# zraorg/ZRA

Hardware: AMD Instinct MI355X
Metric: compress + RA-decompress GiB/s, 16 GiB @ 64 KiB frames, 1/2/4/8 MI355X (higher is better)
Workload: dtype u8

## Files before the change

zra_amd/csrc/zra_encode.hip:

```cpp
#include <cstdio>
#include <unistd.h>
#include "zra_host.h"
#include "zra_dev.h"
#include "zra_format.h"
#include "zra_env.h"
#include <algorithm>
#include <cstdlib>
#include <vector>

extern "C" __global__ void zra_mf_kernel(ZraEncArgs a, uint32_t block, uint32_t only, uint32_t onlySlot, uint32_t perWave);
extern "C" __global__ void zra_mf_opt_kernel(ZraEncArgs a, uint32_t block, uint32_t only, uint32_t onlySlot, uint32_t perWave);
extern "C" __global__ void zra_mf_dfast_ls_kernel(ZraEncArgs a, uint32_t block, uint32_t only, uint32_t onlySlot);
extern "C" __global__ void zra_mf_hc_kernel(ZraEncArgs a, uint32_t block, uint32_t only, uint32_t onlySlot);
extern "C" __global__ void zra_mf_fast_kernel(ZraEncArgs a, uint32_t block, uint32_t perWave);
extern "C" __global__ void zra_mf_dfast_kernel(ZraEncArgs a, uint32_t block, uint32_t only, uint32_t onlySlot);
extern "C" __global__ void zra_mf_dfast_fl_kernel(ZraEncArgs a, ZraFlagArgs g, uint32_t block, uint32_t only, uint32_t onlySlot);
extern "C" __global__ void zra_entropy_kernel(ZraEncArgs a, uint32_t block);
extern "C" __global__ void zra_entropy_front_kernel(ZraEncArgs a, uint32_t block);
extern "C" __global__ void zra_entropy_back_kernel(ZraEncArgs a, uint32_t block);
extern "C" __global__ void zra_ent_chain_kernel(ZraEncArgs a);
extern "C" __global__ void zra_ent_chain5_kernel(ZraEncArgs a);

using namespace zra_dev;
using namespace zra_env;
// ... 147 lines not shown
      if (!encScan_.reserve(64)) return zerr(64);
      bool okProbe = hipMemsetAsync(encScan_.p, 0, 64, stream2_) == hipSuccess &&
                     hipStreamWaitValue32(stream2_, encScan_.p, 0, hipStreamWaitValueGte, 0xFFFFFFFFu) == hipSuccess &&
                     hipStreamSynchronize(stream2_) == hipSuccess;
      if (!okProbe) (void)hipGetLastError();
      waitValueOk_ = okProbe ? 1 : -1;
    }
    if (waitValueOk_ < 0) persist = false;
    if (persist)
      return compress_persistent(dIn, inSize, dBody, bodyBase0, dEntries, dSizes, bodySize, frameSize, checksum, full, tail,
                                 tableWords, seqStride, litStride, slotStride);
  }
  uint64_t budget = 8ull << 30;
  if (env_set("ZRA_ENC_BUDGET_GIB")) budget = (uint64_t)env_int("ZRA_ENC_BUDGET_GIB", 0) << 30;
  else if (full.strategy != 2) {
    size_t freeB = 0, totalB = 0;
    uint64_t mine = 0; for (auto& x : encCtx_) mine += x.tables.cap + x.seqs.cap + x.lits.cap + x.slots.cap;
    if (hipMemGetInfo(&freeB, &totalB) == hipSuccess) budget = std::min<uint64_t>(64ull << 30, std::max<uint64_t>(budget, (uint64_t)(((uint64_t)freeB + mine) * 0.25)));
  }
  uint32_t B = (uint32_t)std::max<uint64_t>(1, std::min<uint64_t>({nFramesTotal, budget / perFrame, full.strategy == 2 ? 16384ull : 65536ull}));
  if (B > 1024) B &= ~1023u;
  { uint64_t nBatches = (nFramesTotal + B - 1) / B;
    if (maxBlocksPerFrame > 1 && nBatches == 1 && nFramesTotal >= 32ull * (uint64_t)numCUs_) nBatches = 2;
    if (nBatches > 1) B = (uint32_t)std::min<uint64_t>(B, ((nFramesTotal + nBatches - 1) / nBatches + 63) & ~63ull); }
  const uint32_t entGridB = (uint32_t)std::min<uint64_t>(B, (uint64_t)numCUs_ * 5);
  const uint64_t entWorkStride = (9 * seqStride + 255) & ~255ull;
  const int nCtx = nFramesTotal > B ? 2 : 1;
  for (int c = 0; c < nCtx; c++) {
    EncCtx& x = encCtx_[c];
    if (!x.tables.reserve(B * tableWords * 4) || !x.seqs.reserve(B * seqStride * 8) || !x.lits.reserve((size_t)entGridB * litStride) ||
        !x.work.reserve((size_t)entGridB * entWorkStride) ||
        !x.slots.reserve(B * slotStride) || !x.misc.reserve(B * (sizeof(ZraEncFrameState) + sizeof(ZraEncBlockOut))) ||
        !x.ck.reserve((size_t)B * 4) || !x.sizes.reserve((size_t)B * 16))
      return zerr(64);
  }
  const size_t nEntLaunches = (size_t)((nFramesTotal + B - 1) / B) * maxBlocksPerFrame + 4;
  if (!encScan_.reserve(64 + 4 * nEntLaunches)) return zerr(64);
  uint64_t* dRunning = encScan_.as<uint64_t>();
  uint32_t* dEntQueues = (uint32_t*)(encScan_.as<uint8_t>() + 64);
  HIPCHK(hipMemsetAsync(encScan_.p, 0, 64 + 4 * nEntLaunches, stream2_));
  size_t entLaunch = 0;

  ZraEncArgs base{};
  base.in = dIn; base.inSize = inSize; base.frameSize = frameSize; base.checksum = checksum ? 1 : 0;
  base.full = full; base.tail = tail;
  dbgSeqStride_ = seqStride; dbgB_ = (uint32_t)B;
  base.tableStride = tableWords; base.seqStride = seqStride; base.litStride = litStride; base.slotStride = slotStride;
  base.entWorkStride = entWorkStride; base.slotRing = B; base.entSubFrames = B; base.entPrio = 3;

  size_t evNext = 0;
  auto ev = [&]() -> hipEvent_t {
    if (evNext == evPool_.size()) { hipEvent_t e = nullptr; if (hipEventCreate(&e) != hipSuccess) return nullptr; evPool_.push_back(e); }
    return evPool_[evNext++];
  };
  std::vector<std::pair<hipEvent_t, hipEvent_t>> mfSpans, entSpans;
  hipEvent_t entDone[2] = {nullptr, nullptr};
  hipStream_t mfStream2 = nullptr;
  if (nCtx == 2) {
    if (!pipeStreams_[0] && hipStreamCreateWithFlags(&pipeStreams_[0], hipStreamNonBlocking) != hipSuccess) { pipeStreams_[0] = nullptr; (void)hipGetLastError(); }
    mfStream2 = pipeStreams_[0];
  }
  { hipEvent_t e0 = ev(); if (!e0) return zerr(1); HIPCHK(hipEventRecord(e0, stream_)); HIPCHK(hipStreamWaitEvent(stream2_, e0, 0));
    if (mfStream2) HIPCHK(hipStreamWaitEvent(mfStream2, e0, 0)); }

  uint64_t batchIdx = 0;
  for (uint64_t f0 = 0; f0 < nFramesTotal; f0 += B, batchIdx++) {
    const uint32_t nb = (uint32_t)std::min<uint64_t>(B, nFramesTotal - f0);
    const int c = (int)(batchIdx % nCtx);
    EncCtx& x = encCtx_[c];
    ZraEncArgs a = base;
    a.firstFrame = (uint32_t)f0; a.nFrames = nb;
    a.tables = x.tables.as<uint32_t>(); a.seqs = x.seqs.as<uint64_t>(); a.lits = x.lits.as<uint8_t>(); a.slots = x.slots.as<uint8_t>();
    a.state = x.misc.as<ZraEncFrameState>();
    a.blockOut = (ZraEncBlockOut*)(x.misc.as<uint8_t>() + (size_t)B * sizeof(ZraEncFrameState));
    a.contentCk = x.ck.as<uint32_t>();
    a.sizes = x.sizes.as<uint64_t>();
    uint64_t* dOffsets = x.sizes.as<uint64_t>() + B;
    if (checksum)
      hipLaunchKernelGGL(zra_content_ck_kernel, dim3((nb * 4 + 255) / 256), dim3(256), 0, stream2_, dIn, (u64)inSize, frameSize, (u32)f0, nb, a.contentCk);
    const uint64_t firstFrameSize = std::min<uint64_t>(frameSize, inSize - f0 * frameSize);
    const ZraEncParams& P0 = firstFrameSize == frameSize ? full : tail;
    const uint32_t rounds = (uint32_t)((firstFrameSize + P0.blockSize - 1) / P0.blockSize);
    hipStream_t sA = (c == 1 && mfStream2) ? mfStream2 : stream_;
    if (entDone[c]) HIPCHK(hipStreamWaitEvent(sA, entDone[c], 0));
    { static const bool poison = env_set("ZRA_ENC_POISON");
      if (poison) HIPCHK(hipMemsetAsync(x.tables.p, 0xA5, (size_t)nb * tableWords * 4, sA)); }
    for (uint32_t blk = 0; blk < rounds; blk++) {
      hipEvent_t m0 = ev(), m1 = ev(), e1 = ev();
      if (!m0 || !m1 || !e1) return zerr(1);
      HIPCHK(hipEventRecord(m0, sA));
      {
        const bool hasTail = tailSize && f0 + nb == nFramesTotal;
        const uint32_t shL = 1, shS = 2, dupLog = 8;
        a.mfFilter = shL | (shS << 4) | (dupLog << 8);
        const uint32_t hl = std::max(full.hashLog, tail.hashLog), cl = std::max(full.chainLog, tail.chainLog);
        const size_t filterBytes = (8u << dupLog) + (((size_t)1 << hl) >> shL) / 8 + (((size_t)1 << cl) >> shS) / 8 + 64;
        const bool serialAll = std::min<uint64_t>(frameSize, inSize) > (1ull << full.windowLog);
        a.serialAll = serialAll ? 1u : 0u;
        const bool oddTail = !serialAll && hasTail && (tail.strategy == 2) != (full.strategy == 2);
        auto launchLone = [&](uint32_t only, uint32_t slot) {
          if (tail.strategy >= 3 && tail.strategy <= 5) hipLaunchKernelGGL(zra_mf_hc_kernel, dim3(1), dim3(64), 0, sA, a, blk, only, slot);
          else hipLaunchKernelGGL(mfGeneric, dim3(1), dim3(64), 0, sA, a, blk, only, slot, 1u);
        };
        if (full.strategy == 2 && !serialAll) {
          hipLaunchKernelGGL(zra_mf_dfast_kernel, dim3(nb), dim3(64), filterBytes, sA, a, blk, 0xFFFFFFFFu, 0u);
          if (oddTail) launchLone((uint32_t)(nb - 1), (uint32_t)(nb - 1));
        } else {
          const bool hashChain = full.strategy >= 3 && full.strategy <= 5 && !serialAll;
          const uint32_t perWave = hashChain ? 1u : std::min<uint32_t>(8u, std::max<uint32_t>(1u, (nb + (uint32_t)numCUs_ * 32 - 1) / ((uint32_t)numCUs_ * 32)));
          const bool lean = hashChain || full.strategy == 1;
          const uint32_t hcPad = hashChain && full.searchLog >= 5 && tableWords * 4 >= (4ull << 20) ? 5120u : 0u;
          if (hashChain) hipLaunchKernelGGL(zra_mf_hc_kernel, dim3(nb), dim3(64), hcPad, sA, a, blk, 0xFFFFFFFFu, 0u);
          else if (lean) hipLaunchKernelGGL(zra_mf_fast_kernel, dim3((nb + perWave - 1) / perWave), dim3(64), 0, sA, a, blk, perWave);
          else hipLaunchKernelGGL(mfGeneric, dim3((nb + perWave - 1) / perWave), dim3(64), 0, sA, a, blk, 0xFFFFFFFFu, 0u, perWave);
          if (oddTail) hipLaunchKernelGGL(zra_mf_dfast_kernel, dim3(1), dim3(64), filterBytes, sA, a, blk, (uint32_t)(nb - 1), (uint32_t)(nb - 1));
          else if (lean && hasTail && (hashChain ? (tail.strategy < 3 || tail.strategy > 5) : tail.strategy != 1))
            launchLone((uint32_t)(nb - 1), (uint32_t)(nb - 1));
        }
      }
      HIPCHK(hipEventRecord(m1, sA));
      mfSpans.push_back({m0, m1});
      HIPCHK(hipStreamWaitEvent(stream2_, m1, 0));
      hipEvent_t e0 = ev(); if (!e0) return zerr(1);
      HIPCHK(hipEventRecord(e0, stream2_));
      { ZraEncArgs ae = a; ae.entQueue = dEntQueues + entLaunch++; ae.entWork = x.work.as<uint8_t>();
        hipLaunchKernelGGL(zra_entropy_kernel, dim3(std::min<uint32_t>(nb, entGridB)), dim3(256), 0, stream2_, ae, blk); }
      HIPCHK(hipEventRecord(e1, stream2_));
      entSpans.push_back({e0, e1});
      if (blk + 1 < rounds) HIPCHK(hipStreamWaitEvent(sA, e1, 0));
    }
    hipLaunchKernelGGL(zra_scan_sizes_kernel, dim3(1), dim3(64), 0, stream2_, a.sizes, nb, dOffsets, dRunning, (const u32*)nullptr);
    hipLaunchKernelGGL(zra_gather_frames_kernel, dim3(nb), dim3(256), 0, stream2_, a.slots, slotStride, a.sizes, dOffsets, dBody,
                       bodyBase0, dEntries ? dEntries : nullptr, (u32)f0, dSizes, (const u32*)nullptr);
    hipEvent_t done = ev(); if (!done) return zerr(1);
    HIPCHK(hipEventRecord(done, stream2_));
    entDone[c] = done;
    if ((uint64_t)env_i64("ZRA_ENC_FAIL_BATCH", -1) == batchIdx) return zerr(1);
  }
  uint64_t total = 0;
  HIPCHK(hipMemcpyAsync(&total, dRunning, 8, hipMemcpyDeviceToHost, stream2_));
  HIPCHK(hipStreamSynchronize(stream2_));
  HIPCHK(hipStreamSynchronize(stream_));
  if (mfStream2) HIPCHK(hipStreamSynchronize(mfStream2));
  HIPCHK(hipGetLastError());
  double kernelMs = 0;
  kstats_[0] = kstats_[1] = kstats_[2] = kstats_[3] = 0;
  for (auto& sp : mfSpans) { float m = 0; if (hipEventElapsedTime(&m, sp.first, sp.second) == hipSuccess) { kstats_[0] += m; kstats_[1] += 1; kernelMs += m; } }
  for (auto& sp : entSpans) { float m = 0; if (hipEventElapsedTime(&m, sp.first, sp.second) == hipSuccess) { kstats_[2] += m; kstats_[3] += 1; } }
  lastKernelMs_ = kernelMs;
  *bodySize = total;
  return ok();
}

Status Engine::compress_persistent(const uint8_t* dIn, size_t inSize, uint8_t* dBody, uint64_t bodyBase0, uint8_t* dEntries, uint64_t* dSizes,
                                   size_t* bodySize, uint32_t frameSize, bool checksum, const ZraEncParams& full, const ZraEncParams& tail,
                                   uint64_t tableWords, uint64_t seqStride, uint64_t litStride, uint64_t slotStride) {
  const uint64_t nFramesTotal = (inSize + frameSize - 1) / frameSize;
  const size_t tailSize = inSize % frameSize;
  const auto mfGeneric = (full.strategy >= 7 || tail.strategy >= 7) ? zra_mf_opt_kernel : zra_mf_kernel;
  static const uint32_t wavesPerCU = (uint32_t)env_int("ZRA_MF_WAVES", 19);
  constexpr uint32_t SB = 8192;
  const uint32_t nSlots = (uint32_t)std::min<uint64_t>((uint64_t)numCUs_ * wavesPerCU, nFramesTotal);
  const uint64_t perFrame = seqStride * 8 + sizeof(ZraEncFrameState) + sizeof(ZraEncBlockOut) + 4 + 16 + 8;
  uint64_t budget;
  {
    size_t freeB = 0, totalB = 0;
    if (hipMemGetInfo(&freeB, &totalB) != hipSuccess) freeB = 24ull << 30;
    uint64_t mine = 0; for (auto& x : encCtx_) mine += x.seqs.cap;
    budget = std::min<uint64_t>(64ull << 30, std::max<uint64_t>(8ull << 30, ((uint64_t)freeB + mine) / 3));
  }
  uint64_t SBIG = 0, nSuper = 0, subsPerSuper = 0; int nCtx = 1;
  EncCtx& sh = encCtx_[0];
  static const uint32_t entPerCU = (uint32_t)std::max(1, env_int("ZRA_ENT_WGS", 8));
  const uint32_t entGrid = (uint32_t)std::min<uint64_t>((uint64_t)numCUs_ * entPerCU, nFramesTotal);
  const uint64_t entWorkStride = (9 * seqStride + 255) & ~255ull;
  static const int splitEnv = env_int("ZRA_ENT_SPLIT", 1);
  const bool entSplit = splitEnv >= 2 || (splitEnv == 1 && nFramesTotal >= 256);
  uint64_t slotRing = 0;
  for (;; budget /= 2) {
    SBIG = std::max<uint64_t>(1, std::min<uint64_t>(nFramesTotal, budget / perFrame));
    if (SBIG > SB) SBIG -= SBIG % SB;
    nCtx = nFramesTotal > SBIG ? 2 : 1;
    nSuper = (nFramesTotal + SBIG - 1) / SBIG;
    subsPerSuper = (SBIG + SB - 1) / SB;
    slotRing = std::min<uint64_t>(SB, SBIG);
    const uint64_t workUnits = entSplit ? std::min<uint64_t>(SB, nFramesTotal) : entGrid;
    bool okR = sh.tables.reserve((size_t)nSlots * tableWords * 4) && sh.lits.reserve((size_t)entGrid * litStride) && sh.work.reserve((size_t)workUnits * entWorkStride) &&
               sh.slots.reserve(slotRing * slotStride) && (!entSplit || sh.rec.reserve((size_t)workUnits * sizeof(ZraEntRec)));
    for (int c = 0; c < nCtx && okR; c++) {
      EncCtx& x = encCtx_[c];
      okR = x.seqs.reserve(SBIG * seqStride * 8) && x.misc.reserve(SBIG * (sizeof(ZraEncFrameState) + sizeof(ZraEncBlockOut))) &&
            x.ck.reserve((size_t)SBIG * 4) && x.sizes.reserve((size_t)SBIG * 16);
    }
    if (okR) break;
    if (budget <= (1ull << 30) || SBIG <= SB) return zerr(64);
    (void)hipGetLastError();
  }
  const size_t nCnt = 4 + 8 * (size_t)nSuper + 4 * (size_t)(nSuper * subsPerSuper) + 4;
  const size_t cntCore = (16 + 4 * nCnt + 15) & ~(size_t)15;
  const size_t cntBytes = cntCore + 8 * (size_t)ZRA_TELE_WORDS;
  if (!encScan_.reserve(cntBytes)) return zerr(64);
  uint64_t* dRunning = encScan_.as<uint64_t>();
  uint32_t* dCnt = (uint32_t*)(encScan_.as<uint8_t>() + 16);
  uint32_t* dPerSuper = dCnt + 4;
  uint32_t* dPerSub = dPerSuper + 8 * nSuper;
  HIPCHK(hipMemsetAsync(encScan_.as<uint8_t>(), 0, cntBytes, stream_));
  encCounters_ = dCnt; encCountersBytes_ = 4 * (4 + 8 * (size_t)nSuper + 4 * (size_t)(nSuper * subsPerSuper));

  ZraEncArgs base{};
  base.in = dIn; base.inSize = inSize; base.frameSize = frameSize; base.checksum = checksum ? 1 : 0;
  base.full = full; base.tail = tail;
  dbgSeqStride_ = seqStride; dbgB_ = (uint32_t)SBIG;
  base.tableStride = tableWords; base.seqStride = seqStride; base.litStride = litStride; base.slotStride = slotStride;
  base.mfTele = (uint64_t*)(encScan_.as<uint8_t>() + cntCore);
  base.entWorkStride = entWorkStride;
  base.entPrio = 1;
  base.entSubFrames = SB; base.slotRing = (uint32_t)slotRing; base.readyStamp = 1u;
  const uint32_t shL = 1, shS = 3, dupLog = 8;
  base.mfFilter = shL | (shS << 4) | (dupLog << 8);
  const uint32_t hl = std::max(full.hashLog, tail.hashLog), cl = std::max(full.chainLog, tail.chainLog);
  const size_t filterBytes = (8u << dupLog) + (((size_t)1 << hl) >> shL) / 8 + (((size_t)1 << cl) >> shS) / 8;

  static const int lsEnv = env_int("ZRA_MF_LS", 1);
  const uint32_t lsBytes = (uint32_t)((std::min<uint64_t>(frameSize, inSize) + 64 + 63) & ~63ull);
  const uint32_t lsPerCu = (uint32_t)((160u << 10) / (lsBytes + filterBytes));
  static const int lsMaxEnv = env_int("ZRA_MF_LS_MAX", -1);
  bool useLs = lsEnv != 0 && full.strategy == 2 && lsPerCu >= 1 &&
               nFramesTotal <= (lsMaxEnv >= 0 ? (uint64_t)lsMaxEnv : (uint64_t)lsPerCu * (uint64_t)numCUs_);
  if (useLs && lsAttr_ == 0) {
    const bool okA = hipFuncSetAttribute((const void*)zra_mf_dfast_ls_kernel, hipFuncAttributeMaxDynamicSharedMemorySize, 160 << 10) == hipSuccess;
    if (!okA) (void)hipGetLastError();
    lsAttr_ = okA ? 1 : -1;
  }
  if (lsAttr_ < 0) useLs = false;

  static const int flEnv = env_int("ZRA_MF_FLAGS", 1);
  const bool useFlagsWave = flEnv != 0 && !useLs && full.strategy == 2;
  ZraFlagArgs fw{};
  if (useFlagsWave) {
    fw.flagStride = ((((uint64_t)std::min<uint64_t>(frameSize, inSize) + 511) / 512) * 128 + 255) & ~255ull;
    if (!mfFlags_.reserve((size_t)nSlots * fw.flagStride)) return zerr(64);
    fw.flags = mfFlags_.as<uint8_t>(); fw.ldsWords = (uint32_t)(filterBytes / 4);
    fw.spanBytes = 768;
    static const int epEnv = env_int("ZRA_MF_EPOCH", 4);
    const uint32_t ibMax = 32u - (uint32_t)__builtin_clz((uint32_t)std::max<uint64_t>(2, std::min<uint64_t>(frameSize, inSize)) - 1u);
    fw.epochBits = (uint32_t)std::max(0, std::min(epEnv, (int)(32u - ibMax) - 10));
  }
  const size_t spanLds = fw.spanBytes ? fw.spanBytes + 16 + (fw.spanBytes / 64 + 1) * 16 : 0;

  size_t evNext = 0;
  auto ev = [&]() -> hipEvent_t {
    if (evNext == evPool_.size()) { hipEvent_t e = nullptr; if (hipEventCreate(&e) != hipSuccess) return nullptr; evPool_.push_back(e); }
    return evPool_[evNext++];
  };
  std::vector<std::pair<hipEvent_t, hipEvent_t>> mfSpans, entSpans;
  static const bool traceOn = env_set("ZRA_ENC_TRACE");
  hipEvent_t superDone[2] = {nullptr, nullptr};
  { hipEvent_t e0 = ev(); if (!e0) return zerr(1); HIPCHK(hipEventRecord(e0, stream_)); HIPCHK(hipStreamWaitEvent(stream2_, e0, 0)); }

  for (uint64_t S = 0; S < nSuper; S++) {
    const uint64_t F0 = S * SBIG;
    const uint32_t n = (uint32_t)std::min<uint64_t>(SBIG, nFramesTotal - F0);
    const int c = (int)(S % nCtx);
    EncCtx& x = encCtx_[c];
    ZraEncArgs a = base;
    a.firstFrame = (uint32_t)F0; a.nFrames = n;
    a.tables = sh.tables.as<uint32_t>(); a.lits = sh.lits.as<uint8_t>(); a.slots = sh.slots.as<uint8_t>(); a.entWork = sh.work.as<uint8_t>();
    a.seqs = x.seqs.as<uint64_t>();
    a.state = x.misc.as<ZraEncFrameState>();
    a.blockOut = (ZraEncBlockOut*)(x.misc.as<uint8_t>() + (size_t)SBIG * sizeof(ZraEncFrameState));
    a.contentCk = x.ck.as<uint32_t>();
    a.sizes = x.sizes.as<uint64_t>();
    a.mfQueue = dPerSuper + 8 * S; a.mfStarted = a.mfQueue + 1;
    uint32_t* const entQ = dPerSub + 4 * S * subsPerSuper;
    a.mfDone = entQ + 3 * subsPerSuper;
    if (superDone[c]) HIPCHK(hipStreamWaitEvent(stream_, superDone[c], 0));
    HIPCHK(hipMemsetAsync(a.blockOut, 0, (size_t)n * sizeof(ZraEncBlockOut), stream_));
    hipEvent_t m0 = ev(), m1 = ev();
    if (!m0 || !m1) return zerr(1);
    HIPCHK(hipEventRecord(m0, stream_));
    const uint32_t mfGrid = std::min<uint32_t>(n, nSlots);
    if (useFlagsWave) hipLaunchKernelGGL(zra_mf_dfast_fl_kernel, dim3(mfGrid), dim3(64), filterBytes + spanLds, stream_, a, fw, 0u, 0xFFFFFFFFu, 0u);
    else if (useLs) {
      ZraEncArgs al = a; al.mfFilter |= (lsBytes / 64) << 16;
      hipLaunchKernelGGL(zra_mf_dfast_ls_kernel, dim3(mfGrid), dim3(64), lsBytes + filterBytes, stream_, al, 0u, 0xFFFFFFFFu, 0u);
    } else hipLaunchKernelGGL(zra_mf_dfast_kernel, dim3(mfGrid), dim3(64), filterBytes, stream_, a, 0u, 0xFFFFFFFFu, 0u);
    HIPCHK(hipGetLastError());
    HIPCHK(hipEventRecord(m1, stream_));
    mfSpans.push_back({m0, m1});
    const bool oddTail = tailSize && F0 + n == nFramesTotal && tail.strategy != 2;
    if (oddTail) {
      ZraEncArgs at = a; at.mfQueue = nullptr;
      if (tail.strategy >= 3 && tail.strategy <= 5) hipLaunchKernelGGL(zra_mf_hc_kernel, dim3(1), dim3(64), 0, stream_, at, 0u, (uint32_t)(n - 1), 0u);
      else hipLaunchKernelGGL(mfGeneric, dim3(1), dim3(64), 0, stream_, at, 0u, (uint32_t)(n - 1), 0u, 1u);
    }
    HIPCHK(hipStreamWaitValue32(stream2_, a.mfStarted, mfGrid, hipStreamWaitValueGte, 0xFFFFFFFFu));
    if (checksum)
      hipLaunchKernelGGL(zra_content_ck_kernel, dim3((n * 4 + 255) / 256), dim3(256), 0, stream2_, dIn, (u64)inSize, frameSize, (u32)F0, n, a.contentCk);
    const uint32_t nSub1 = (n + SB - 1) / SB;
    for (uint32_t j = 0; j < nSub1; j++) {
      const uint32_t j0 = j * SB, nbj = std::min<uint32_t>(SB, n - j0);
      const bool hasOdd = oddTail && j == nSub1 - 1;
      HIPCHK(hipStreamWaitValue32(stream2_, a.mfDone + j, nbj - (hasOdd ? 1u : 0u), hipStreamWaitValueGte, 0xFFFFFFFFu));
      if (hasOdd) { hipEvent_t te = ev(); if (!te) return zerr(1); HIPCHK(hipEventRecord(te, stream_)); HIPCHK(hipStreamWaitEvent(stream2_, te, 0)); }
      ZraEncArgs aj = a;
      aj.firstFrame = (uint32_t)(F0 + j0); aj.nFrames = nbj;
      aj.seqs = a.seqs + (size_t)j0 * seqStride; aj.state = a.state + j0; aj.blockOut = a.blockOut + j0;
      aj.contentCk = a.contentCk + j0; aj.sizes = a.sizes + j0;
      aj.entQueue = entQ + j;
      uint64_t* dOffsets = x.sizes.as<uint64_t>() + SBIG + j0;
      hipEvent_t e0 = ev(), e1 = ev(); if (!e0 || !e1) return zerr(1);
      HIPCHK(hipEventRecord(e0, stream2_));
      if (entSplit) {
        aj.entRec = sh.rec.as<ZraEntRec>();
        hipLaunchKernelGGL(zra_entropy_front_kernel, dim3(std::min<uint32_t>(nbj, entGrid)), dim3(256), 0, stream2_, aj, 0u);
        const uint32_t cg = wavesPerCU >= 19 ? 5u : 6u;
        hipLaunchKernelGGL(cg == 5 ? zra_ent_chain5_kernel : zra_ent_chain_kernel, dim3((nbj + cg - 1) / cg), dim3(64), 0, stream2_, aj);
        ZraEncArgs ab = aj; ab.entQueue = entQ + subsPerSuper + j;
        hipLaunchKernelGGL(zra_entropy_back_kernel, dim3(std::min<uint32_t>(nbj, entGrid)), dim3(256), 0, stream2_, ab, 0u);
      } else
        hipLaunchKernelGGL(zra_entropy_kernel, dim3(std::min<uint32_t>(nbj, entGrid)), dim3(256), 0, stream2_, aj, 0u);
      HIPCHK(hipEventRecord(e1, stream2_));
      entSpans.push_back({e0, e1});
      hipLaunchKernelGGL(zra_scan_sizes_kernel, dim3(1), dim3(64), 0, stream2_, aj.sizes, nbj, dOffsets, dRunning, (const u32*)nullptr);
      hipLaunchKernelGGL(zra_gather_frames_kernel, dim3(nbj), dim3(256), 0, stream2_, aj.slots, slotStride, aj.sizes, dOffsets, dBody,
                         bodyBase0, dEntries ? dEntries : nullptr, (u32)(F0 + j0), dSizes, (const u32*)nullptr);
    }
    hipEvent_t done = ev(); if (!done) return zerr(1);
    HIPCHK(hipEventRecord(done, stream2_));
    superDone[c] = done;
  }
  uint64_t total = 0;
  HIPCHK(hipMemcpyAsync(&total, dRunning, 8, hipMemcpyDeviceToHost, stream2_));
  HIPCHK(hipStreamSynchronize(stream2_));
  HIPCHK(hipStreamSynchronize(stream_));
  HIPCHK(hipGetLastError());
  double kernelMs = 0;
  kstats_[0] = kstats_[1] = kstats_[2] = kstats_[3] = 0;
  for (auto& sp : mfSpans) { float m = 0; if (hipEventElapsedTime(&m, sp.first, sp.second) == hipSuccess) { kstats_[0] += m; kstats_[1] += 1; kernelMs += m; } }
  for (auto& sp : entSpans) { float m = 0; if (hipEventElapsedTime(&m, sp.first, sp.second) == hipSuccess) { kstats_[2] += m; kstats_[3] += 1; } }
  lastKernelMs_ = kernelMs;
  mfTeleDev_ = base.mfTele;
  if (traceOn) {
    for (auto& sp : mfSpans) { float a0 = 0, a1 = 0; (void)hipEventElapsedTime(&a0, mfSpans[0].first, sp.first); (void)hipEventElapsedTime(&a1, mfSpans[0].first, sp.second); std::fprintf(stderr, "mf  %8.2f .. %8.2f ms\n", a0, a1); }
    for (auto& sp : entSpans) { float a0 = 0, a1 = 0; (void)hipEventElapsedTime(&a0, mfSpans[0].first, sp.first); (void)hipEventElapsedTime(&a1, mfSpans[0].first, sp.second); std::fprintf(stderr, "ent %8.2f .. %8.2f ms\n", a0, a1); }
  }
  *bodySize = total;
  return ok();
}

size_t Engine::launch_telemetry(uint64_t* out, size_t cap) {
  if (mfTeleDev_) {
    (void)hipSetDevice(device_);
    mfTele_.resize(ZRA_TELE_HEAD + 8 + ZRA_TELE_CUKEYS);
    const bool okT = hipMemcpy(mfTele_.data(), mfTeleDev_, 8 * (size_t)ZRA_TELE_HEAD, hipMemcpyDeviceToHost) == hipSuccess &&
                     hipMemcpy(mfTele_.data() + ZRA_TELE_HEAD, mfTeleDev_ + ZRA_TELE_ENT, 8 * (size_t)(8 + ZRA_TELE_CUKEYS), hipMemcpyDeviceToHost) == hipSuccess;
    if (!okT) { (void)hipGetLastError(); mfTele_.clear(); }
    mfTeleDev_ = nullptr;
  }
  const size_t n = mfTele_.size() < cap ? mfTele_.size() : cap;
  for (size_t i = 0; i < n; i++) out[i] = mfTele_[i];
  return n;
}

uint32_t Engine::debug_read_seqs(uint32_t frame, uint64_t* out, uint32_t cap, uint32_t meta[3]) {
  if (!dbgB_ || frame >= dbgB_) return 0;
  (void)hipSetDevice(device_);
  (void)hipDeviceSynchronize();
  EncCtx& x = encCtx_[0];
  ZraEncBlockOut bo{};
  (void)hipMemcpy(&bo, x.misc.as<uint8_t>() + (size_t)dbgB_ * sizeof(ZraEncFrameState) + (size_t)frame * sizeof(ZraEncBlockOut), sizeof(bo), hipMemcpyDeviceToHost);
  meta[0] = bo.nbSeq; meta[1] = bo.lastLL; meta[2] = bo.skip;
  const uint32_t n = bo.nbSeq < cap ? bo.nbSeq : cap;
  if (n) (void)hipMemcpy(out, x.seqs.as<uint64_t>() + (size_t)frame * dbgSeqStride_, (size_t)n * 8, hipMemcpyDeviceToHost);
  return n;
}

Status Engine::compress_device(const uint8_t* dIn, size_t inSize, uint8_t* dOut, size_t* outSize, int level, uint32_t frameSize, bool checksum) {
  HIPCHK(hipSetDevice(device_));
  if (frameSize == 0) return zerr(42);
  const uint32_t tableSize = zra_fmt::table_size(inSize, frameSize);
  const size_t headerSize = zra_fmt::kFixedSize + (size_t)tableSize * zra_fmt::kEntrySize;
  size_t bodySize = 0;
  Status s = compress_impl(dIn, inSize, dOut + headerSize, 0, dOut + zra_fmt::kFixedSize, nullptr, &bodySize, level, frameSize, checksum);
  if (s.zra) return s;
  if (headerSize + bodySize >= zra_fmt::kMaxCompressedSize) return {kCompressedTooLarge, 0};
  std::vector<uint8_t> hdr(headerSize);
  if (tableSize > 1)
    HIPCHK(hipMemcpyAsync(hdr.data() + zra_fmt::kFixedSize, dOut + zra_fmt::kFixedSize, (size_t)(tableSize - 1) * 5, hipMemcpyDeviceToHost, stream_));
  HIPCHK(hipStreamSynchronize(stream_));
  zra_fmt::write_fixed(hdr.data(), inSize, tableSize, frameSize, 0);
  zra_fmt::entry_put(hdr.data() + zra_fmt::kFixedSize + (size_t)(tableSize - 1) * 5, bodySize);
  zra_fmt::wr32(hdr.data() + 14, zra_fmt::header_hash(hdr.data(), hdr.data() + zra_fmt::kFixedSize));
  HIPCHK(hipMemcpyAsync(dOut, hdr.data(), zra_fmt::kFixedSize, hipMemcpyHostToDevice, stream_));
  HIPCHK(hipMemcpyAsync(dOut + zra_fmt::kFixedSize + (size_t)(tableSize - 1) * 5, hdr.data() + zra_fmt::kFixedSize + (size_t)(tableSize - 1) * 5, 5,
                        hipMemcpyHostToDevice, stream_));
  HIPCHK(hipStreamSynchronize(stream_));
  *outSize = headerSize + bodySize;
  return ok();
}

// ... 21 lines not shown
```

zra_amd/csrc/zra_encode_mf.hip:

```cpp
#include "zra_dev.h"
#include "zra_kernels.h"
#include "zra_encode_wave.h"

using namespace zra_dev;
using namespace zra_wave;

#ifdef ZRA_MF_PROFILE
__device__ unsigned long long zra_mf_prof[24];
#define PROF_DECL u64 pt_[20]; for (int k_ = 0; k_ < 20; k_++) pt_[k_] = 0; u64 pl_ = __builtin_amdgcn_s_memtime();
#define PROF(k) { __builtin_amdgcn_s_waitcnt(0); const u64 n_ = __builtin_amdgcn_s_memtime(); pt_[k] += n_ - pl_; pl_ = n_; }
#define PROF_CNT(k) { pt_[k]++; }
#define PROF_END { if (lane == 0) for (int k_ = 0; k_ < 20; k_++) atomicAdd(&zra_mf_prof[k_], pt_[k_]); }
#elif defined(ZRA_MF_MARK)
#define PROF_DECL
#define PROF(k) asm volatile("; ZMARK " #k);
#define PROF_CNT(k)
#define PROF_END
#else
#define PROF_DECL
#define PROF(k)
#define PROF_CNT(k)
#define PROF_END
#endif

// ... 886 lines not shown
            const u32 mr = wave_count_eq(src, ip + 4, ip + 4 - o1, be, lane) + 4;
            const int g2 = (int)(mr * 3), g1 = (int)(ml * 3 - hb32(off + 1) + 1);
            if (mr >= 4 && g2 > g1) { ml = mr; off = 0; start = ip; }
          }
          {
            m2 = search(ip, oc2);
            const int g2 = (int)(m2 * 4 - hb32(oc2 + 1)), g1 = (int)(ml * 4 - hb32(off + 1) + 4);
            if (m2 >= 4 && g2 > g1) { ml = m2; off = oc2; start = ip; continue; }
          }
          if (depth == 2 && ip < ilimit) {
            ip++;
            if (off && o1 > 0 && rep_test(ip, true)) {
              const u32 mr = wave_count_eq(src, ip + 4, ip + 4 - o1, be, lane) + 4;
              const int g2 = (int)(mr * 4), g1 = (int)(ml * 4 - hb32(off + 1) + 1);
              if (mr >= 4 && g2 > g1) { ml = mr; off = 0; start = ip; }
            }
            {
              m2 = search(ip, oc2);
              const int g2 = (int)(m2 * 4 - hb32(oc2 + 1)), g1 = (int)(ml * 4 - hb32(off + 1) + 7);
              if (m2 >= 4 && g2 > g1) { ml = m2; off = oc2; start = ip; continue; }
            }
          }
          break;
        }
      }
      if (off) {
        const u32 ro = off - 2;
        const u32 back = (start > ro) ? wave_count_back(src, start, start - ro, anchor, lane) : 0u;
        start -= back; ml += back;
        o2 = o1; o1 = ro;
      }
    }
    put(start - anchor, ml, off ? off + 1 : 1);
    anchor = ip = start + ml;
    while (ip <= ilimit && o2 > 0 && rep_test(ip, false)) {
      const u32 rl = wave_count_eq(src, ip + 4, ip + 4 - o2, be, lane) + 4;
      const u32 t = o2; o2 = o1; o1 = t;
      put(0, rl, 1);
      ip += rl; anchor = ip;
    }
  }
  rep[0] = o1 ? o1 : saved; rep[1] = o2 ? o2 : saved;
  *nOut = n;
#ifdef ZRA_MF_PROFILE
  HPROF(2) HCNT(4, n) HCNT(5, 1)
  if (lane == 0) for (int k_ = 0; k_ < 12; k_++) atomicAdd(&zra_mf_prof[k_], H.pt[k_]);
#endif
  return be - anchor;
}

}

struct MfFrame {
  const ZraEncParams* P; const u8* src; ZraEncFrameState* st; ZraEncBlockOut* bo; u32* hashT; u32* chainT; u64* seqs;
  u32 fsize, bs, be;
};
__device__ __forceinline__ bool mf_frame_setup(const ZraEncArgs& a, u32 block, int lane, MfFrame& F, u32 f, u32 tableSlot, bool hcwOnly = false, bool keepTables = false) {
  const u64 fstart = (u64)(a.firstFrame + f) * a.frameSize;
  const u64 remaining = a.inSize - fstart;
  F.fsize = (u32)(remaining < a.frameSize ? remaining : a.frameSize);
  F.P = (F.fsize == a.frameSize) ? &a.full : &a.tail;
  const u32 blockSize = F.P->blockSize;
  F.bs = block * blockSize;
  if (F.bs >= F.fsize && !(F.fsize == 0 && block == 0)) return false;
  F.be = min(F.fsize, F.bs + blockSize);
  F.src = a.in + fstart;
  F.st = &a.state[f];
  F.hashT = a.tables + (size_t)tableSlot * a.tableStride;
  F.chainT = F.hashT + ((size_t)1 << F.P->hashLog);
  F.bo = &a.blockOut[f];
  F.seqs = a.seqs + (size_t)f * a.seqStride;
  if (block == 0) {
    size_t words = (size_t)1 << F.P->hashLog;
    if (!hcwOnly) words += (size_t)1 << F.P->chainLog;
    if (F.P->strategy >= 7)
      words += (F.P->minMatch == 3 ? (size_t)1 << min(17u, F.P->windowLog) : 0) + 512;
    if (keepTables) words = 0;
    uint4* t4 = (uint4*)F.hashT;
    for (size_t i = lane; i < words / 4; i += 64) t4[i] = make_uint4(0, 0, 0, 0);
    for (size_t i = (words / 4) * 4 + lane; i < words; i += 64) F.hashT[i] = 0;
    if (lane == 0) { F.st->rep[0] = 1; F.st->rep[1] = 4; F.st->rep[2] = 8; F.st->nextToUpdate = 1; F.st->insEnd = 1; F.st->idxShift = 0; }
    __builtin_amdgcn_fence(__ATOMIC_RELEASE, "workgroup");
    __builtin_amdgcn_wave_barrier();
    __builtin_amdgcn_fence(__ATOMIC_ACQUIRE, "workgroup");
  }
  if (F.be - F.bs < 7) {
    if (lane == 0) { F.bo->nbSeq = 0; F.bo->lastLL = F.be - F.bs; F.bo->skip = 1; }
    return false;
  }
  return true;
}

template <int MODE>
__device__ __forceinline__ void mf_serial_block_t(const MfFrame& F, u32 ntu0) {
  const ZraEncParams& P = *F.P;
  const u8* src = F.src; ZraEncFrameState* st = F.st; ZraEncBlockOut* bo = F.bo;
  u32* hashT = F.hashT; u32* chainT = F.chainT;
  const u32 bs = F.bs, be = F.be;
  u32 rep[3] = {st->rep[0], st->rep[1], st->rep[2]};
  u32 lastLL;
  bo->skip = 0;
  Emit E; E.seqs = F.seqs; E.n = 0;
  u32 ntu = ntu0;
  { const u32 cur = bs + 1; if (cur > ntu + 384) { const u32 d = cur - ntu - 384; ntu = cur - (d < 192 ? d : 192); } }
  if constexpr (MODE == 1) lastLL = mf_fast(P, hashT, src, bs, be, rep, E);
  else if (MODE == 0 && P.strategy >= 7) {
    OptCtx O;
    O.hashT = hashT; O.bt = chainT; O.hashLog = P.hashLog; O.chainLog = P.chainLog; O.searchLog = P.searchLog;
    O.minMatchParam = P.minMatch; O.targetLength = P.targetLength; O.lvl = P.strategy == 7 ? 0 : 2; O.windowLog = P.windowLog;
    O.hashLog3 = P.minMatch == 3 ? min(17u, P.windowLog) : 0;
    O.hash3 = chainT + ((size_t)1 << P.chainLog);
    O.o = (ZraOptState*)(O.hash3 + (O.hashLog3 ? (size_t)1 << O.hashLog3 : 0));
    O.idxShift = st->idxShift;
    ntu = ntu0;
    { const u32 cur = bs + 1 + O.idxShift; if (cur > ntu + 384) { const u32 d = cur - ntu - 384; ntu = cur - (d < 192 ? d : 192); } }
    O.nextToUpdate = ntu;
    if (P.strategy == 9 && O.o->litLengthSum == 0 && bs == 0 && ntu == 1 && be - bs > 1024) {
      u32 tmpRep[3] = {rep[0], rep[1], rep[2]};
      (void)O.parse(src, bs, be, tmpRep, E, true);
      O.idxShift += be - bs;
      O.nextToUpdate = 1 + O.idxShift;
      O.upscale_stats();
    }
    lastLL = O.parse(src, bs, be, rep, E, false);
    ntu = O.nextToUpdate;
    st->idxShift = O.idxShift;
  } else if (P.strategy == 1) lastLL = mf_fast(P, hashT, src, bs, be, rep, E);
  else if (P.strategy == 2) lastLL = mf_dfast_serial(P, hashT, chainT, src, bs, be, rep, E);
  else {
    HC H; H.hashT = hashT; H.chainT = chainT; H.hlog = P.hashLog; H.mls = P.minMatch < 4 ? 4 : P.minMatch > 6 ? 6 : P.minMatch;
    H.chainSize = 1u << P.chainLog; H.cmask = H.chainSize - 1; H.searchLog = P.searchLog; H.nextToUpdate = ntu;
    H.windowLog = P.windowLog;
    H.bt = P.strategy == 6;
    lastLL = mf_lazy(H, src, bs, be, rep, E, P.strategy == 6 ? 2 : (int)P.strategy - 3);
    ntu = H.nextToUpdate;
  }
  st->nextToUpdate = ntu; st->insEnd = ntu;
  bo->nbSeq = E.n; bo->lastLL = lastLL;
  bo->rep[0] = rep[0]; bo->rep[1] = rep[1]; bo->rep[2] = rep[2];
}

struct DfBlock { u64 a; u64 m; };
__device__ __forceinline__ DfBlock df_block_load(const u8* src, u32 fsize, const u8* flg, u32 blk, bool haveMasks, int lane) {
  DfBlock B; B.a = 0; B.m = 0;
  const u32 c = blk * 512 + 8 * (u32)lane;
  if (c + 8 <= fsize) B.a = ld64(src + c);
  else if (c < fsize) B.a = ld64_safe(src + c, src + fsize);
  if (haveMasks && lane < 16) B.m = *(const u64*)(flg + (size_t)blk * 128 + 8 * (u32)lane);
  return B;
}
__device__ __forceinline__ void df_later_flags(const u8* src, u32 fsize, u32 hlog, u32 clog, u32 mls, u32* lds, u32 ldsWords, u8* flg, int lane) {
  if (fsize < 8) return;
  const u32 lastPos = fsize - 8;
  const u32 bmWords = ldsWords - 128;
  u32 npLog = 0;
  while ((((1u << hlog) + (1u << clog)) >> npLog) > bmWords * 32) npLog++;
  const u32 hlogP = hlog - npLog, clogP = clog - npLog;
  u32* const cnt = lds; u32* const bmL = lds + 128; u32* const bmS = bmL + ((1u << hlogP) >> 5);
  const u64 primeS = mls == 5 ? 889523592379ULL : mls == 6 ? 227718039650203ULL : 58295818150454627ULL;
  const u32 shV = 64 - 8 * min(mls, 7u);
  const u32 nBlk = lastPos / 512 + 1;
  const u32 srcLane = (u32)lane >> 3, sh = ((u32)lane & 7u) * 8;
  for (u32 pass = 0; pass < (1u << npLog); pass++) {
    for (u32 i = (u32)lane; i < 128 + ((1u << hlogP) >> 5) + ((1u << clogP) >> 5); i += 64) lds[i] = 0;
    __builtin_amdgcn_fence(__ATOMIC_ACQ_REL, "workgroup");
    const bool hm = pass != 0;
    DfBlock B0 = df_block_load(src, fsize, flg, nBlk - 1, hm, lane), B1{0, 0};
    u64 above = nBlk * 512 < fsize ? ld64_safe(src + nBlk * 512, src + fsize) : 0;
    for (u32 blk = nBlk; blk-- > 0;) {
      if (blk >= 1) B1 = df_block_load(src, fsize, flg, blk - 1, hm, lane);
      const u32 aLo = (u32)B0.a, aHi = (u32)(B0.a >> 32);
      u64 outM = 0;
#pragma unroll 1
      for (u32 kk = 0; kk < 4; kk++) {
        if (blk * 512 + (6 - 2 * kk) * 64 > lastPos) continue;
        u32 iLw[2], iSw[2]; bool pLw[2], pSw[2];
#pragma unroll
        for (int h = 0; h < 2; h++) {
          const u32 k = 7 - 2 * kk - h;
          const u32 p = blk * 512 + k * 64 + (u32)lane;
          const bool act = p <= lastPos;
          const u32 ci = 8 * k + srcLane;
          const u32 c0l = (u32)__builtin_amdgcn_ds_bpermute((int)(4 * ci), (int)aLo), c0h = (u32)__builtin_amdgcn_ds_bpermute((int)(4 * ci), (int)aHi);
          u32 c1l = (u32)__builtin_amdgcn_ds_bpermute((int)(4 * ((ci + 1) & 63)), (int)aLo), c1h = (u32)__builtin_amdgcn_ds_bpermute((int)(4 * ((ci + 1) & 63)), (int)aHi);
          if (ci == 63) { c1l = (u32)above; c1h = (u32)(above >> 32); }
          const u64 c0 = (u64)c0l | ((u64)c0h << 32), c1 = (u64)c1l | ((u64)c1h << 32);
          const u64 v = sh ? (c0 >> sh) | (c1 << (64 - sh)) : c0;
          const u32 bL = (u32)((v * 0xCF1BBCDCB7A56463ULL) >> (64 - hlog));
          const u32 bS = mls <= 4 ? ((u32)v * 2654435761u) >> (32 - clog) : (u32)(((v << shV) * primeS) >> (64 - clog));
          pLw[h] = act && (bL >> hlogP) == pass; pSw[h] = act && (bS >> clogP) == pass;
          iLw[h] = bL & ((1u << hlogP) - 1); iSw[h] = bS & ((1u << clogP) - 1);
        }
        u32 seenL[2], seenS[2], cL[2], cS[2];
#pragma unroll
        for (int h = 0; h < 2; h++) {
          const u32 iL = iLw[h], iS = iSw[h], sL = iL & 255u, sS = 256u + (iS & 255u);
          const bool pL = pLw[h], pS = pSw[h];
          seenL[h] = pL ? lds_read32(&bmL[iL >> 5]) : 0u; seenS[h] = pS ? lds_read32(&bmS[iS >> 5]) : 0u;
          if (pL) atomicAdd(&cnt[sL >> 2], 1u << (8 * (sL & 3)));
          if (pS) atomicAdd(&cnt[sS >> 2], 1u << (8 * (sS & 3)));
          __builtin_amdgcn_wave_barrier();
          cL[h] = pL ? lds_read32(&cnt[sL >> 2]) : 0u;
          cS[h] = pS ? lds_read32(&cnt[sS >> 2]) : 0u;
          __builtin_amdgcn_wave_barrier();
          if (pL) { atomicSub(&cnt[sL >> 2], 1u << (8 * (sL & 3))); atomicOr(&bmL[iL >> 5], 1u << (iL & 31)); }
          if (pS) { atomicSub(&cnt[sS >> 2], 1u << (8 * (sS & 3))); atomicOr(&bmS[iS >> 5], 1u << (iS & 31)); }
          __builtin_amdgcn_wave_barrier();
        }
#pragma unroll
        for (int h = 0; h < 2; h++) {
          const u32 k = 7 - 2 * kk - h;
          if (blk * 512 + k * 64 > lastPos) continue;
          const u32 iL = iLw[h], iS = iSw[h], sL = iL & 255u, sS = iS & 255u;
          const u64 mL = __ballot(((seenL[h] >> (iL & 31)) & 1u) || ((cL[h] >> (8 * (sL & 3))) & 255u) > 1);
          const u64 mS = __ballot(((seenS[h] >> (iS & 31)) & 1u) || ((cS[h] >> (8 * (sS & 3))) & 255u) > 1);
          if ((u32)lane == 2 * k) outM = mL;
          if ((u32)lane == 2 * k + 1) outM = mS;
        }
      }
      if (lane < 16) *(u64*)(flg + (size_t)blk * 128 + 8 * (u32)lane) = outM | B0.m;
      above = (u64)bcast(aLo, 0) | ((u64)bcast(aHi, 0) << 32);
      B0 = B1;
    }
    __builtin_amdgcn_fence(__ATOMIC_RELEASE, "agent");
    __builtin_amdgcn_fence(__ATOMIC_ACQUIRE, "agent");
  }
}
template <bool FLAGS, bool LSRC = false>
__device__ __forceinline__ void mf_dfast_body(const ZraEncArgs& a, u32 block, u32 only, u32 onlySlot, const ZraFlagArgs* g = nullptr) {
  const int lane = threadIdx.x;
  extern __shared__ u32 dynLds[];
  LeanLds W;
  W.shL = a.mfFilter & 15; W.shS = (a.mfFilter >> 4) & 15; W.dupSlots = 1u << ((a.mfFilter >> 8) & 15);
  u32* const fltLds = LSRC ? dynLds + (a.mfFilter >> 16) * 16 : dynLds;
  W.dup = (u8*)fltLds;
  W.bmL = fltLds + 2 * W.dupSlots;
  W.span = nullptr; W.spanFlg = nullptr; W.spanBytes = 0;
  if (FLAGS && g && g->spanBytes) { W.spanBytes = g->spanBytes; W.span = (u8*)(fltLds + g->ldsWords); W.spanFlg = W.span + g->spanBytes + 16; }
  const bool persistent = a.mfQueue != nullptr;
  const bool tele = persistent && a.mfTele != nullptr;
  u64* const tl = tele ? a.mfTele + ZRA_TELE_HEAD + 4 * (size_t)min(blockIdx.x, ZRA_TELE_WAVES - 1u) : nullptr;
  if (tele && lane == 0) {
    const u32 hw = __builtin_amdgcn_s_getreg((31 << 11) | 4);
    const u32 xcc = __builtin_amdgcn_s_getreg((3 << 11) | 20) & 7u;
    const u64 tc0 = __builtin_readcyclecounter(), tr0 = wall_clock64();
    const u32 key = (xcc << 8) | (((hw >> 13) & 7u) << 5) | (((hw >> 12) & 1u) << 4) | ((hw >> 8) & 15u);
    atomicAdd((unsigned long long*)&a.mfTele[32 + key], 1ull << (16u * ((hw >> 4) & 3u)));
    atomicAdd((unsigned long long*)&a.mfTele[8 + xcc], 1ull);
    atomicMax((unsigned long long*)&a.mfTele[4], ~tr0);
    atomicMax((unsigned long long*)&a.mfTele[6], tr0);
    tl[0] = tc0; tl[1] = tr0; tl[2] = xcc; tl[3] = 0;
  }
  if (persistent && a.mfStarted && lane == 0) atomicAdd(a.mfStarted, 1u);
  const u32 epochBits = (FLAGS && g && persistent) ? min(g->epochBits, ZRA_DF_EPOCH_BITS) : 0u;
  u32 epochCtr = 0;
  for (;;) {
    u32 f = only == 0xFFFFFFFFu ? blockIdx.x : only;
    if (persistent) {
      u32 t = 0;
      if (lane == 0) t = atomicAdd(a.mfQueue, 1u);
      f = rfl(t);
      if (f >= a.nFrames) {
        if (tele && lane == 0) {
          const u64 tc1 = __builtin_readcyclecounter(), tr1 = wall_clock64();
          const u64 tc0 = tl[0], tr0 = tl[1];
          const u32 xcc = (u32)tl[2] & 7u;
          atomicAdd((unsigned long long*)&a.mfTele[0], tc1 - tc0);
          atomicAdd((unsigned long long*)&a.mfTele[1], tr1 - tr0);
          atomicAdd((unsigned long long*)&a.mfTele[2], 1ull);
          atomicMax((unsigned long long*)&a.mfTele[3], tr1 - tr0);
          atomicMax((unsigned long long*)&a.mfTele[5], tr1);
          atomicMax((unsigned long long*)&a.mfTele[7], ~tr1);
          atomicAdd((unsigned long long*)&a.mfTele[16 + xcc], (unsigned long long)tl[3]);
          atomicAdd((unsigned long long*)&a.mfTele[24 + xcc], tr1 - tr0);
        }
        return;
      }
      if (tele && lane == 0) tl[3]++;
    }
#ifdef ZRA_MF_PROFILE
    const u64 kt0_ = __builtin_amdgcn_s_memtime();
#endif
    bool mine = true;
    {
      const u64 fstart = (u64)(a.firstFrame + f) * a.frameSize;
      const ZraEncParams& Pf = (a.inSize - fstart < a.frameSize) ? a.tail : a.full;
      if (Pf.strategy != 2) mine = false;
    }
    MfFrame F;
    bool keepTables = false; u32 epoch = 0;
    if (epochBits && mine) {
      const u64 fstart = (u64)(a.firstFrame + f) * a.frameSize;
      const bool fullFrame = a.inSize - fstart >= a.frameSize;
      if (!fullFrame) epochCtr = 0;
      epoch = epochCtr & ((1u << epochBits) - 1u);
      keepTables = epoch != 0;
      epochCtr = fullFrame ? epochCtr + 1 : 0;
    }
    if (mine && mf_frame_setup(a, block, lane, F, f, persistent ? blockIdx.x : only == 0xFFFFFFFFu ? f : onlySlot, false, keepTables)) {
#ifdef ZRA_MF_PROFILE
      __builtin_amdgcn_s_waitcnt(0);
      if (lane == 0) atomicAdd(&zra_mf_prof[20], __builtin_amdgcn_s_memtime() - kt0_);
#endif
      const u32 wordsL = ((1u << F.P->hashLog) >> W.shL) / 32, wordsS = ((1u << F.P->chainLog) >> W.shS) / 32;
      W.bmS = W.bmL + wordsL;
      u32 rep[3] = {F.st->rep[0], F.st->rep[1], F.st->rep[2]};
      u32 lastLL, nseq = 0;
      const u32 ib = 32 - __builtin_clz(F.fsize - 1);
      const u8* flg = nullptr;
      if (FLAGS && g && g->flags && block == 0 && persistent) {
        u8* const fw = g->flags + (size_t)blockIdx.x * g->flagStride;
        df_later_flags(F.src, F.fsize, F.P->hashLog, F.P->chainLog, F.P->minMatch, fltLds, g->ldsWords, fw, lane);
        flg = fw;
      }
      {
        const u32 fill = block == 0 ? 0u : 0xFFFFFFFFu;
        for (u32 i = lane; i < wordsL + wordsS; i += 64) W.bmL[i] = fill;
        __builtin_amdgcn_fence(__ATOMIC_ACQ_REL, "workgroup");
      }
      const u8* srcP = F.src;
      if (LSRC) {
        u8* const ls = (u8*)dynLds;
        const u32 n16 = F.fsize >> 4;
        for (u32 i = (u32)lane; i < n16; i += 64) *(uint4*)(ls + 16 * i) = ld128(F.src + 16 * i);
        for (u32 i = (n16 << 4) + (u32)lane; i < F.fsize; i += 64) ls[i] = F.src[i];
        ls[F.fsize + (u32)lane] = 0;
        __builtin_amdgcn_fence(__ATOMIC_RELEASE, "workgroup");
        __builtin_amdgcn_wave_barrier();
        __builtin_amdgcn_fence(__ATOMIC_ACQUIRE, "workgroup");
        srcP = ls;
      }
      switch (F.P->minMatch) {
        case 5: lastLL = mf_dfast_lean<5, FLAGS>(*F.P, F.hashT, F.chainT, srcP, F.bs, F.be, rep, F.seqs, &nseq, W, lane, ib, flg, epoch); break;
        case 6: lastLL = mf_dfast_lean<6, FLAGS>(*F.P, F.hashT, F.chainT, srcP, F.bs, F.be, rep, F.seqs, &nseq, W, lane, ib, flg, epoch); break;
        case 7: lastLL = mf_dfast_lean<7, FLAGS>(*F.P, F.hashT, F.chainT, srcP, F.bs, F.be, rep, F.seqs, &nseq, W, lane, ib, flg, epoch); break;
        default: lastLL = mf_dfast_lean<4, FLAGS>(*F.P, F.hashT, F.chainT, srcP, F.bs, F.be, rep, F.seqs, &nseq, W, lane, ib, flg, epoch); break;
      }
      if (lane == 0) {
        F.bo->nbSeq = nseq; F.bo->lastLL = lastLL; F.bo->skip = 0;
        F.bo->rep[0] = rep[0]; F.bo->rep[1] = rep[1]; F.bo->rep[2] = rep[2];
      }
#ifdef ZRA_MF_PROFILE
      __builtin_amdgcn_s_waitcnt(0);
      if (lane == 0) { atomicAdd(&zra_mf_prof[21], __builtin_amdgcn_s_memtime() - kt0_); atomicAdd(&zra_mf_prof[22], 1ull); }
#endif
    }
    if (!persistent) return;
    if (mine) {
      __builtin_amdgcn_fence(__ATOMIC_RELEASE, "agent");
      if (lane == 0) { __hip_atomic_store(&a.blockOut[f].ready, a.readyStamp, __ATOMIC_RELEASE, __HIP_MEMORY_SCOPE_AGENT); if (a.mfDone) atomicAdd(&a.mfDone[f / a.entSubFrames], 1u); }
    }
  }
}

extern "C" __global__ void __launch_bounds__(64)
zra_mf_dfast_kernel(ZraEncArgs a, u32 block, u32 only, u32 onlySlot) { mf_dfast_body<false>(a, block, only, onlySlot); }
extern "C" __global__ void __launch_bounds__(64) __attribute__((amdgpu_waves_per_eu(6)))
zra_mf_dfast_fl_kernel(ZraEncArgs a, ZraFlagArgs g, u32 block, u32 only, u32 onlySlot) { mf_dfast_body<true>(a, block, only, onlySlot, &g); }
// ... 101 lines not shown
```

Before: 20.62.

## Shrink match-finder flag LDS footprint to allow a 20th finder wave per CU

The flag pass now uses one 64-word byte-counter region for both the long-hash and short-hash collision counts, running them one after the other instead of side by side. This halves the counter LDS and leaves more words for the seen-bitmaps. A constexpr geometry helper picks a coarser short-hash shift (shS=4) and drops the span buffer when 20 or more waves per CU are requested, so the filter fits in 5 LDS pieces instead of 6. The default is still 19 waves, so by default only the serialized counter path changes, which adds extra wave barriers per hash step.

```diff
diff --git a/zra_amd/csrc/zra_encode.hip b/zra_amd/csrc/zra_encode.hip
--- a/zra_amd/csrc/zra_encode.hip
+++ b/zra_amd/csrc/zra_encode.hip
@@ -323,6 +323,19 @@
   return ok();
 }
 
+constexpr uint32_t kLdsPiece = 1280;
+struct MfLdsGeometry { uint32_t shL, shS, dupLog, spanBytes; size_t filterBytes; };
+constexpr size_t mf_span_lds(uint32_t spanBytes) { return (size_t)spanBytes + 16 + (spanBytes / 64 + 1) * 16; }
+constexpr size_t mf_filter_bytes(uint32_t hl, uint32_t cl, uint32_t shL, uint32_t shS, uint32_t dupLog) {
+  return ((size_t)8 << dupLog) + (((size_t)1 << hl) >> shL) / 8 + (((size_t)1 << cl) >> shS) / 8;
+}
+constexpr MfLdsGeometry mf_lds_geometry(uint32_t hl, uint32_t cl, uint32_t wavesPerCU) {
+  if (wavesPerCU >= 20 && mf_filter_bytes(hl, cl, 1, 4, 8) <= 5 * kLdsPiece) return MfLdsGeometry{1, 4, 8, 0, mf_filter_bytes(hl, cl, 1, 4, 8)};
+  return MfLdsGeometry{1, 3, 8, 768, mf_filter_bytes(hl, cl, 1, 3, 8)};
+}
+static_assert(mf_lds_geometry(16, 15, 20).spanBytes == 0 && mf_lds_geometry(16, 15, 20).filterBytes <= 5 * kLdsPiece && 20 * 5 + 14 <= 128, "a 20th finder wave needs the 5-piece layout");
+static_assert(mf_lds_geometry(16, 15, 19).filterBytes + mf_span_lds(768) <= 6 * kLdsPiece && 19 * 6 + 14 <= 128, "19 finder waves of 6 pieces fill the CU");
+
 Status Engine::compress_persistent(const uint8_t* dIn, size_t inSize, uint8_t* dBody, uint64_t bodyBase0, uint8_t* dEntries, uint64_t* dSizes,
                                    size_t* bodySize, uint32_t frameSize, bool checksum, const ZraEncParams& full, const ZraEncParams& tail,
                                    uint64_t tableWords, uint64_t seqStride, uint64_t litStride, uint64_t slotStride) {
@@ -387,14 +400,12 @@
   base.entWorkStride = entWorkStride;
   base.entPrio = 1;
   base.entSubFrames = SB; base.slotRing = (uint32_t)slotRing; base.readyStamp = 1u;
-  const uint32_t shL = 1, shS = 3, dupLog = 8;
-  base.mfFilter = shL | (shS << 4) | (dupLog << 8);
   const uint32_t hl = std::max(full.hashLog, tail.hashLog), cl = std::max(full.chainLog, tail.chainLog);
-  const size_t filterBytes = (8u << dupLog) + (((size_t)1 << hl) >> shL) / 8 + (((size_t)1 << cl) >> shS) / 8;
+  const size_t lsFilterBytes = mf_lds_geometry(hl, cl, 0).filterBytes;
 
   static const int lsEnv = env_int("ZRA_MF_LS", 1);
   const uint32_t lsBytes = (uint32_t)((std::min<uint64_t>(frameSize, inSize) + 64 + 63) & ~63ull);
-  const uint32_t lsPerCu = (uint32_t)((160u << 10) / (lsBytes + filterBytes));
+  const uint32_t lsPerCu = (uint32_t)((160u << 10) / (lsBytes + lsFilterBytes));
   static const int lsMaxEnv = env_int("ZRA_MF_LS_MAX", -1);
   bool useLs = lsEnv != 0 && full.strategy == 2 && lsPerCu >= 1 &&
                nFramesTotal <= (lsMaxEnv >= 0 ? (uint64_t)lsMaxEnv : (uint64_t)lsPerCu * (uint64_t)numCUs_);
@@ -407,17 +418,20 @@
 
   static const int flEnv = env_int("ZRA_MF_FLAGS", 1);
   const bool useFlagsWave = flEnv != 0 && !useLs && full.strategy == 2;
+  const MfLdsGeometry geo = mf_lds_geometry(hl, cl, useFlagsWave ? wavesPerCU : 0);
+  base.mfFilter = geo.shL | (geo.shS << 4) | (geo.dupLog << 8);
+  const size_t filterBytes = geo.filterBytes;
   ZraFlagArgs fw{};
   if (useFlagsWave) {
     fw.flagStride = ((((uint64_t)std::min<uint64_t>(frameSize, inSize) + 511) / 512) * 128 + 255) & ~255ull;
     if (!mfFlags_.reserve((size_t)nSlots * fw.flagStride)) return zerr(64);
     fw.flags = mfFlags_.as<uint8_t>(); fw.ldsWords = (uint32_t)(filterBytes / 4);
-    fw.spanBytes = 768;
+    fw.spanBytes = geo.spanBytes;
     static const int epEnv = env_int("ZRA_MF_EPOCH", 4);
     const uint32_t ibMax = 32u - (uint32_t)__builtin_clz((uint32_t)std::max<uint64_t>(2, std::min<uint64_t>(frameSize, inSize)) - 1u);
     fw.epochBits = (uint32_t)std::max(0, std::min(epEnv, (int)(32u - ibMax) - 10));
   }
-  const size_t spanLds = fw.spanBytes ? fw.spanBytes + 16 + (fw.spanBytes / 64 + 1) * 16 : 0;
+  const size_t spanLds = fw.spanBytes ? mf_span_lds(fw.spanBytes) : 0;
 
   size_t evNext = 0;
   auto ev = [&]() -> hipEvent_t {
diff --git a/zra_amd/csrc/zra_encode_mf.hip b/zra_amd/csrc/zra_encode_mf.hip
--- a/zra_amd/csrc/zra_encode_mf.hip
+++ b/zra_amd/csrc/zra_encode_mf.hip
@@ -1062,17 +1062,17 @@
 __device__ __forceinline__ void df_later_flags(const u8* src, u32 fsize, u32 hlog, u32 clog, u32 mls, u32* lds, u32 ldsWords, u8* flg, int lane) {
   if (fsize < 8) return;
   const u32 lastPos = fsize - 8;
-  const u32 bmWords = ldsWords - 128;
+  const u32 bmWords = ldsWords - 64;
   u32 npLog = 0;
   while ((((1u << hlog) + (1u << clog)) >> npLog) > bmWords * 32) npLog++;
   const u32 hlogP = hlog - npLog, clogP = clog - npLog;
-  u32* const cnt = lds; u32* const bmL = lds + 128; u32* const bmS = bmL + ((1u << hlogP) >> 5);
+  u32* const cnt = lds; u32* const bmL = lds + 64; u32* const bmS = bmL + ((1u << hlogP) >> 5);
   const u64 primeS = mls == 5 ? 889523592379ULL : mls == 6 ? 227718039650203ULL : 58295818150454627ULL;
   const u32 shV = 64 - 8 * min(mls, 7u);
   const u32 nBlk = lastPos / 512 + 1;
   const u32 srcLane = (u32)lane >> 3, sh = ((u32)lane & 7u) * 8;
   for (u32 pass = 0; pass < (1u << npLog); pass++) {
-    for (u32 i = (u32)lane; i < 128 + ((1u << hlogP) >> 5) + ((1u << clogP) >> 5); i += 64) lds[i] = 0;
+    for (u32 i = (u32)lane; i < 64 + ((1u << hlogP) >> 5) + ((1u << clogP) >> 5); i += 64) lds[i] = 0;
     __builtin_amdgcn_fence(__ATOMIC_ACQ_REL, "workgroup");
     const bool hm = pass != 0;
     DfBlock B0 = df_block_load(src, fsize, flg, nBlk - 1, hm, lane), B1{0, 0};
@@ -1104,16 +1104,20 @@
         u32 seenL[2], seenS[2], cL[2], cS[2];
 #pragma unroll
         for (int h = 0; h < 2; h++) {
-          const u32 iL = iLw[h], iS = iSw[h], sL = iL & 255u, sS = 256u + (iS & 255u);
+          const u32 iL = iLw[h], iS = iSw[h], sL = iL & 255u, sS = iS & 255u;
           const bool pL = pLw[h], pS = pSw[h];
           seenL[h] = pL ? lds_read32(&bmL[iL >> 5]) : 0u; seenS[h] = pS ? lds_read32(&bmS[iS >> 5]) : 0u;
           if (pL) atomicAdd(&cnt[sL >> 2], 1u << (8 * (sL & 3)));
+          __builtin_amdgcn_wave_barrier();
+          cL[h] = pL ? lds_read32(&cnt[sL >> 2]) : 0u;
+          __builtin_amdgcn_wave_barrier();
+          if (pL) atomicSub(&cnt[sL >> 2], 1u << (8 * (sL & 3)));
+          __builtin_amdgcn_wave_barrier();
           if (pS) atomicAdd(&cnt[sS >> 2], 1u << (8 * (sS & 3)));
           __builtin_amdgcn_wave_barrier();
-          cL[h] = pL ? lds_read32(&cnt[sL >> 2]) : 0u;
           cS[h] = pS ? lds_read32(&cnt[sS >> 2]) : 0u;
           __builtin_amdgcn_wave_barrier();
-          if (pL) { atomicSub(&cnt[sL >> 2], 1u << (8 * (sL & 3))); atomicOr(&bmL[iL >> 5], 1u << (iL & 31)); }
+          if (pL) atomicOr(&bmL[iL >> 5], 1u << (iL & 31));
           if (pS) { atomicSub(&cnt[sS >> 2], 1u << (8 * (sS & 3))); atomicOr(&bmS[iS >> 5], 1u << (iS & 31)); }
           __builtin_amdgcn_wave_barrier();
         }
```

Measured after the change: 20.63 (median of 2 runs). About the same (+0.0%).
